# DanEngelbrecht/longtail

Hardware: AMD Instinct MI355X
Metric: ingest GB/s (chunk+hash+compress) (higher is better)
Workload: dtype u8/u32

## Files before the change

longtail_amd/csrc/ablations/k_buzhash_prefix_regs.inc:

```

template <int MODE, int WAVES>
__global__ __launch_bounds__(64 * WAVES, 1) void k_buzhash_prefix(const uint8_t* __restrict__ data,
                                                                   const PartDev* __restrict__ parts,
                                                                   const uint32_t* __restrict__ tile_part,
                                                                   uint32_t ntiles, DivTest dv,
                                                                   uint64_t* __restrict__ bm0,
                                                                   uint64_t* __restrict__ bm1)
{
    extern __shared__ __attribute__((aligned(16))) uint32_t smem[];
    const int tid = threadIdx.x;
    const int lane = tid & 63;
    const int wave = __builtin_amdgcn_readfirstlane(tid >> 6);
    uint32_t* rows = smem + 256 * TAB_REP + wave * (WROWS * ROW_DW + HALO_DW);
    uint32_t* halo = rows + WROWS * ROW_DW;
    prefix_table_init(smem, tid, 64 * WAVES);

    const uint32_t rows_byte = (uint32_t)(uintptr_t)(const __attribute__((address_space(3))) uint32_t*)rows;
    PrefixConsts pc;
    pc.lane4 = (uint32_t)lane * 4u;
    pc.hj = 63u - (uint32_t)lane;
    pc.halo_byte = rows_byte + WROWS * ROW_DW * 4u;
    pc.thr = MODE == 1 ? 0u : 0xFFFFFFFFu / (dv.d >> dv.k2);
    pc.exact_add = dv.addc - dv.inv;

    const uint64_t nwt = (uint64_t)ntiles * 4u;
    const uint64_t wstride = (uint64_t)gridDim.x * (uint64_t)WAVES;
    uint64_t wt = (uint64_t)blockIdx.x * (uint64_t)WAVES + (uint64_t)wave;
    if (wt >= nwt)
        return;
    PartDev pd = parts[tile_part[wt >> 2]];
    uint64_t span = ((wt >> 2) - pd.tile_base) * (uint64_t)TILE + (wt & 3u) * (uint64_t)WTILE;
    TileRegs regs;
    tile_load(regs, data, pd, span, lane);

    for (;;)
    {
        __builtin_amdgcn_wave_barrier();
        tile_store(regs, rows, lane);
        __builtin_amdgcn_wave_barrier();

        const uint64_t next = wt + wstride;
        PartDev npd = pd;
        uint64_t next_span = 0;
        if (next < nwt)
        {
            npd = parts[tile_part[next >> 2]];
            next_span = ((next >> 2) - npd.tile_base) * (uint64_t)TILE + (next & 3u) * (uint64_t)WTILE;
            tile_load(regs, data, npd, next_span, lane);
        }

        uint32_t win[16];
        const uint32_t* own = rows + (lane + 1) * ROW_DW;
#pragma unroll
        for (int i = 0; i < 16; ++i)
            win[i] = own[i];
        const uint32_t hb = lds_load_u8(rows_byte + pc.hj);
        const uint64_t m = prefix_legal(prefix_tile<MODE>(win, hb, pc, dv, lane, halo), span + (uint64_t)lane * RUN, pd.size);

        const uint64_t summary = __builtin_amdgcn_ballot_w64(m != 0ull);
        if (m != 0ull)
            bm0[pd.bm0_base + (span >> 6) + (uint64_t)lane] = m;
        if (lane == 0)
            bm1[pd.bm1_base + (span >> 12)] = summary;

        if (next >= nwt)
            break;
        wt = next;
        pd = npd;
        span = next_span;
    }
}
```

longtail_amd/csrc/ablations/k_buzhash_roll.inc:

```

constexpr int K1_WAVES = 12;
constexpr int K1_THREADS = 64 * K1_WAVES;
constexpr int WVECS = WROWS * 4;

struct TileRegs
{
    uint4 q[5];
};

__device__ __forceinline__ void tile_load(TileRegs& r, const uint8_t* __restrict__ data, const PartDev& pd,
                                          uint64_t span_start, int lane)
{
    const uint8_t* src = data + pd.off;
#pragma unroll
    for (int u = 0; u < 5; ++u)
    {
        const int v = lane + u * 64;
        uint4 q = make_uint4(0, 0, 0, 0);
        if (v < WVECS)
        {
            const int64_t g = (int64_t)span_start - 64 + 16 * (int64_t)v;
            if (g >= 0)
            {
                if ((uint64_t)g + 16 <= pd.size)
                    q = *reinterpret_cast<const uint4*>(src + g);
                else if ((uint64_t)g < pd.size)
                {
                    uint32_t w[4] = {0, 0, 0, 0};
                    const uint32_t n = (uint32_t)(pd.size - (uint64_t)g);
                    for (uint32_t b = 0; b < n; ++b)
                        w[b >> 2] |= (uint32_t)src[g + b] << (8 * (b & 3));
                    q = make_uint4(w[0], w[1], w[2], w[3]);
                }
            }
        }
        r.q[u] = q;
    }
}

__device__ __forceinline__ void tile_store(const TileRegs& r, uint32_t* __restrict__ rows, int lane)
{
#pragma unroll
    for (int u = 0; u < 5; ++u)
    {
        const int v = lane + u * 64;
        if (v < WVECS)
        {
            uint32_t* d = rows + (v >> 2) * ROW_DW + (v & 3) * 4;
            d[0] = r.q[u].x;
            d[1] = r.q[u].y;
            d[2] = r.q[u].z;
            d[3] = r.q[u].w;
        }
    }
}

template <int MODE>
__global__ __launch_bounds__(K1_THREADS, 1) void k_buzhash_candidates(const uint8_t* __restrict__ data,
                                                                       const PartDev* __restrict__ parts,
                                                                       const uint32_t* __restrict__ tile_part,
                                                                       uint32_t ntiles, DivTest dv,
                                                                       uint64_t* __restrict__ bm0,
                                                                       uint64_t* __restrict__ bm1)
{
    extern __shared__ __attribute__((aligned(16))) uint32_t smem[];
    uint32_t* tab = smem;

    const int tid = threadIdx.x;
    const int lane = tid & 63;
    const int wave = __builtin_amdgcn_readfirstlane(tid >> 6);
    uint32_t* rows = smem + 256 * TAB_REP + wave * (WROWS * ROW_DW);

    if (tid < 256)
    {
        const uint32_t tv = c_buztab[tid];
        uint4 q = make_uint4(tv, tv, tv, tv);
        uint4* dst = reinterpret_cast<uint4*>(tab + tid * TAB_REP);
#pragma unroll
        for (int j = 0; j < TAB_REP / 4; ++j)
            dst[j] = q;
    }
    __syncthreads();
    if ((uint32_t)(uintptr_t)(const __attribute__((address_space(3))) uint32_t*)smem != 0u)
        __builtin_trap();
    const uint32_t lane4 = (uint32_t)lane * 4u;
    const uint32_t qodd = MODE == 1 ? 0u : 0xFFFFFFFFu / (dv.d >> dv.k2);

    const uint64_t nwt = (uint64_t)ntiles * 4u;
    const uint64_t wstride = (uint64_t)gridDim.x * (uint64_t)K1_WAVES;
    uint64_t wt = (uint64_t)blockIdx.x * (uint64_t)K1_WAVES + (uint64_t)wave;
    if (wt >= nwt)
        return;
    PartDev pd = parts[tile_part[wt >> 2]];
    uint64_t span = ((wt >> 2) - pd.tile_base) * (uint64_t)TILE + (wt & 3u) * (uint64_t)WTILE;
    TileRegs regs;
    tile_load(regs, data, pd, span, lane);

    for (;;)
    {
        __builtin_amdgcn_wave_barrier();
        tile_store(regs, rows, lane);
        __builtin_amdgcn_wave_barrier();

        const uint64_t next = wt + wstride;
        PartDev npd = pd;
        uint64_t next_span = 0;
        if (next < nwt)
        {
            npd = parts[tile_part[next >> 2]];
            next_span = ((next >> 2) - npd.tile_base) * (uint64_t)TILE + (next & 3u) * (uint64_t)WTILE;
            tile_load(regs, data, npd, next_span, lane);
        }

        const uint64_t q0 = span + (uint64_t)lane * RUN;
        uint32_t mlo = 0, mhi = 0;
        if (q0 < pd.size)
        {
            uint32_t win[28];
            const uint32_t* prev = rows + lane * ROW_DW;
#pragma unroll
            for (int i = 0; i < 12; ++i)
                win[i] = prev[4 + i];
#pragma unroll
            for (int i = 0; i < 16; ++i)
                win[12 + i] = prev[ROW_DW + i];

            uint32_t tv[48 + RUN];
            uint32_t h = 0;
#define LT_LOOKUP(j)                                                                                                 \
    tv[j] = lds_load_u32(__builtin_amdgcn_perm(win[(j) >> 2], lane4, 0x0c0c0400u | ((uint32_t)((j) & 3) << 8)))
#define LT_STEP(k)                                                                                                   \
    {                                                                                                                \
        h = rotl32(h, 1) ^ rotl32(tv[k], 16) ^ tv[48 + (k)];                                                         \
        bool pre;                                                                                                    \
        if (MODE == 1)                                                                                               \
            pre = (h & (dv.d - 1u)) == dv.d - 1u;                                                                    \
        else         \
            pre = h * dv.inv + dv.inv <= qodd;                                                                       \
        if (__builtin_amdgcn_ballot_w64(pre) != 0ull)        \
        {                                                                                                            \
            asm volatile("");                  \
            const bool hit = MODE == 1 ? pre : rotr32(h * dv.inv + dv.addc, dv.k2) <= dv.qlim;    \
             \
            uint32_t hb;                                                                                             \
            asm volatile("v_cndmask_b32_e64 %0, 0, 1, %1" : "=v"(hb) : "s"(__builtin_amdgcn_ballot_w64(hit)));       \
            if ((k) < 32)                                                                                            \
                mlo |= hb << (k);                                                                                    \
            else                                                                                                     \
                mhi |= hb << ((k)-32);                                                                               \
        }                                                                                                            \
    }
#pragma unroll
            for (int j = 0; j < 80; ++j)
                LT_LOOKUP(j);
            __builtin_amdgcn_sched_barrier(0);
#pragma unroll
            for (int j = 0; j < 48; ++j)
                h = rotl32(h, 1) ^ tv[j];
#pragma unroll
            for (int k = 0; k < 32; ++k)
                LT_STEP(k)
            __builtin_amdgcn_sched_barrier(0);
#pragma unroll
            for (int j = 80; j < 48 + RUN; ++j)
                LT_LOOKUP(j);
            __builtin_amdgcn_sched_barrier(0);
#pragma unroll
            for (int k = 32; k < RUN; ++k)
                LT_STEP(k)
#undef LT_LOOKUP
#undef LT_STEP
            uint64_t m = ((uint64_t)mhi << 32) | mlo;
            if (q0 < 47)
                m &= ~0ull << (47 - q0);
            const uint64_t remain = pd.size - q0;
            if (remain < 64)
                m &= (1ull << remain) - 1ull;
            mlo = (uint32_t)m;
            mhi = (uint32_t)(m >> 32);
        }
        const uint64_t m = ((uint64_t)mhi << 32) | mlo;
        const uint64_t summary = __builtin_amdgcn_ballot_w64(m != 0ull);
        if (m != 0ull)
            bm0[pd.bm0_base + (span >> 6) + (uint64_t)lane] = m;
        if (lane == 0)
            bm1[pd.bm1_base + (span >> 12)] = summary;

        if (next >= nwt)
            break;
        wt = next;
        pd = npd;
        span = next_span;
    }
}
```

longtail_amd/csrc/k_buzhash.hip:

```cpp
#include "lthip_internal.h"

#include <stdlib.h>
#include <type_traits>

namespace
{

__constant__ uint32_t c_buztab[256] = {
#include "buzhash_table.inc"
};

#include "k_blake3_leaf.h"

constexpr int RUN = 64;
constexpr int TILE = 256 * RUN;
constexpr int ROW_DW = 17;
constexpr int TAB_REP = 64;

__device__ __forceinline__ uint32_t lds_load_u32(uint32_t byte_addr)
{
#if defined(__HIP_DEVICE_COMPILE__)
    return *(const __attribute__((address_space(3))) uint32_t*)byte_addr;
#else
    (void)byte_addr;
    return 0u;
#endif
}

__device__ __forceinline__ uint32_t lds_load_u8(uint32_t byte_addr)
{
#if defined(__HIP_DEVICE_COMPILE__)
    return *(const __attribute__((address_space(3))) uint8_t*)byte_addr;
#else
    (void)byte_addr;
    return 0u;
#endif
}

__device__ __forceinline__ uint4 lds_load_u128(uint32_t byte_addr)
{
#if defined(__HIP_DEVICE_COMPILE__)
    typedef uint32_t v4 __attribute__((ext_vector_type(4)));
    const v4 q = *(const __attribute__((address_space(3))) v4*)byte_addr;
    return make_uint4(q.x, q.y, q.z, q.w);
#else
    (void)byte_addr;
    return make_uint4(0, 0, 0, 0);
#endif
}

__device__ __forceinline__ uint32_t rotl32(uint32_t x, uint32_t r) { return __builtin_amdgcn_alignbit(x, x, (32u - r) & 31u); }
__device__ __forceinline__ uint32_t rotr32(uint32_t x, uint32_t r) { return __builtin_amdgcn_alignbit(x, x, r & 31u); }

__global__ void k_tile_table(const PartDev* __restrict__ parts, uint32_t nparts, uint32_t* __restrict__ tile_part,
                             uint64_t ntiles)
{
    uint64_t t = (uint64_t)blockIdx.x * blockDim.x + threadIdx.x;
    if (t >= ntiles)
        return;
    uint32_t lo = 0, hi = nparts;
    while (hi - lo > 1)
    {
        uint32_t mid = lo + (hi - lo) / 2;
        if ((uint64_t)parts[mid].tile_base <= t)
            lo = mid;
        else
            hi = mid;
    }
    tile_part[t] = lo;
}

constexpr int WROWS = 64 + 1;
constexpr int WTILE = 64 * RUN;

#ifdef LTHIP_ABLATIONS
#include "ablations/k_buzhash_roll.inc"
#endif

#ifndef K1_MAD64
#define K1_MAD64 0
#endif
constexpr int HALO_DW = 64;

struct PrefixConsts
{
    uint32_t lane4;
    uint32_t hj;
    uint32_t halo_byte;
    uint32_t thr;
    uint32_t exact_add;
};

template <int MODE>
__device__ __forceinline__ uint64_t prefix_tile(const uint32_t (&win)[16], uint32_t hb, const PrefixConsts& pc, const DivTest& dv,
                                                int lane, uint32_t* __restrict__ halo)
{
    {
        uint32_t x = lds_load_u32((hb << 8) | pc.lane4);
        x = rotr32(x, pc.hj);
        if (lane >= 47)
            x = 0u;
        x ^= (uint32_t)__builtin_amdgcn_update_dpp(0, (int)x, 0x111, 0xf, 0xf, false);
        x ^= (uint32_t)__builtin_amdgcn_update_dpp(0, (int)x, 0x112, 0xf, 0xf, false);
        x ^= (uint32_t)__builtin_amdgcn_update_dpp(0, (int)x, 0x114, 0xf, 0xf, false);
        x ^= (uint32_t)__builtin_amdgcn_update_dpp(0, (int)x, 0x118, 0xf, 0xf, false);
        x ^= (uint32_t)__builtin_amdgcn_update_dpp(0, (int)x, 0x142, 0xa, 0xf, false);
        x ^= (uint32_t)__builtin_amdgcn_update_dpp(0, (int)x, 0x143, 0xc, 0xf, false);
        halo[pc.hj] = x;
    }

    uint32_t S[65];
#define LT_LOOKUP(j) S[j] = lds_load_u32(__builtin_amdgcn_perm(win[(j) >> 2], pc.lane4, 0x0c0c0400u | ((uint32_t)((j) & 3) << 8)))
#pragma unroll
    for (int j = 63; j >= 0; --j)
        LT_LOOKUP(j);
#undef LT_LOOKUP
    __builtin_amdgcn_sched_barrier(0);
    S[64] = 0u;
#pragma unroll
    for (int j = 63; j >= 0; --j)
        S[j] = S[j + 1] ^ ((j & 31) ? rotr32(S[j], (uint32_t)(j & 31)) : S[j]);
    __builtin_amdgcn_wave_barrier();

    uint32_t mlo = 0, mhi = 0;
    uint32_t inv_v;
    asm volatile("v_mov_b32 %0, %1" : "=v"(inv_v) : "s"(dv.inv));
#if K1_MAD64
    const uint64_t inv64 = (uint64_t)inv_v;
#endif
    typedef uint32_t u32x4 __attribute__((ext_vector_type(4)));
    u32x4 Q[16];
    auto halo_quad = [&](auto QI) __attribute__((always_inline))
    {
        constexpr int q = decltype(QI)::value;
        if constexpr (q >= 4 && q <= 15)
        {
            u32x4 v = {S[4 * q], S[4 * q + 1], S[4 * q + 2], S[4 * q + 3]};
            uint64_t save;
            asm volatile("s_mov_b64 %[sv], exec\n\ts_mov_b64 exec, %[msk]\n\t"
                         "ds_read_b128 %[r], %[ad] offset:%[o]\n\t"
                         "s_mov_b64 exec, %[sv]"
                         : [sv] "=&s"(save), [r] "+v"(v)
                         : [ad] "v"(pc.halo_byte), [msk] "s"(0x8000000000000000ull), [o] "i"(16 * q)
                         : "memory");
            Q[q] = v;
        }
    };
    auto halo_wait = [&](auto QI) __attribute__((always_inline))
    {
        constexpr int q = decltype(QI)::value;
        if constexpr (q >= 4 && q <= 15)
        {
            u32x4 v = Q[q];
            if constexpr (q >= 6)
                asm volatile("s_waitcnt lgkmcnt(2)" : "+v"(v));
            else if constexpr (q == 5)
                asm volatile("s_waitcnt lgkmcnt(1)" : "+v"(v));
            else
                asm volatile("s_waitcnt lgkmcnt(0)" : "+v"(v));
            S[4 * q] = v.x;
            S[4 * q + 1] = v.y;
            S[4 * q + 2] = v.z;
            S[4 * q + 3] = v.w;
        }
    };
    auto group = [&](auto G) __attribute__((always_inline))
    {
        constexpr int g = decltype(G)::value;
        uint32_t y[8];
#pragma unroll
        for (int half = 1; half >= 0; --half)
        {
            if (half == 1)
                halo_wait(std::integral_constant<int, 2 * g + 1 + 4>{});
            else
                halo_wait(std::integral_constant<int, 2 * g + 4>{});
#pragma unroll
            for (int ii = 3; ii >= 0; --ii)
            {
                const int i = 4 * half + ii;
                const int k = 8 * g + i;
                uint32_t w;
                if (k >= 47)
                    w = S[k - 47] ^ S[k + 1];
                else
                    w = (S[0] ^ S[k + 1]) ^ (uint32_t)__builtin_amdgcn_update_dpp(0, (int)S[(k + 17) & 63], 0x13C, 0xf, 0xf, false);
                const uint32_t h = (k & 31) ? rotl32(w, (uint32_t)(k & 31)) : w;
                if (MODE == 1)
                    y[i] = ~h & (dv.d - 1u);
                else
                {
#if K1_MAD64
                    uint64_t t, carry;
                    asm("v_mad_u64_u32 %0, %1, %2, %3, %4" : "=v"(t), "=s"(carry) : "v"(h), "s"(dv.inv), "v"(inv64));
                    y[i] = (uint32_t)t;
#else
                    y[i] = h * dv.inv + inv_v;
#endif
                }
            }
            if (half == 1)
                halo_quad(std::integral_constant<int, 2 * g + 2>{});
            else
                halo_quad(std::integral_constant<int, 2 * g + 1>{});
        }
        const uint32_t m = min(min(min(y[0], y[1]), y[2]), min(min(min(y[3], y[4]), y[5]), min(y[6], y[7])));
        if (__builtin_amdgcn_ballot_w64(m <= pc.thr) != 0ull)
        {
            asm volatile("");
#pragma unroll
            for (int i = 0; i < 8; ++i)
            {
                const int k = 8 * g + i;
                if (__builtin_amdgcn_ballot_w64(y[i] <= pc.thr) != 0ull)
                {
                    asm volatile("");
                    const bool hit = MODE == 1 ? y[i] == 0u : rotr32(y[i] + pc.exact_add, dv.k2) <= dv.qlim;
                    uint32_t hbit;
                    asm volatile("v_cndmask_b32_e64 %0, 0, 1, %1" : "=v"(hbit) : "s"(__builtin_amdgcn_ballot_w64(hit)));
                    if (k < 32)
                        mlo |= hbit << k;
                    else
                        mhi |= hbit << (k - 32);
                }
            }
        }
    };
    group(std::integral_constant<int, 7>{});
    group(std::integral_constant<int, 6>{});
    group(std::integral_constant<int, 5>{});
    group(std::integral_constant<int, 4>{});
    group(std::integral_constant<int, 3>{});
    group(std::integral_constant<int, 2>{});
    group(std::integral_constant<int, 1>{});
    group(std::integral_constant<int, 0>{});
    return ((uint64_t)mhi << 32) | mlo;
}

__device__ __forceinline__ uint64_t prefix_legal(uint64_t m, uint64_t q0, uint64_t size)
{
    if (q0 >= size)
        return 0ull;
    if (q0 < 47)
        m &= ~0ull << (47 - q0);
    const uint64_t remain = size - q0;
    if (remain < 64)
        m &= (1ull << remain) - 1ull;
    return m;
}

__device__ __forceinline__ void prefix_table_init(uint32_t* tab, int tid, int nthreads)
{
    for (int v = tid; v < 256; v += nthreads)
    {
        const uint32_t tv = c_buztab[v];
        uint4 q = make_uint4(tv, tv, tv, tv);
        uint4* dst = reinterpret_cast<uint4*>(tab + v * TAB_REP);
#pragma unroll
        for (int j = 0; j < TAB_REP / 4; ++j)
            dst[j] = q;
    }
    __syncthreads();
    if ((uint32_t)(uintptr_t)(const __attribute__((address_space(3))) uint32_t*)tab != 0u)
        __builtin_trap();
}

#ifdef LTHIP_ABLATIONS
#include "ablations/k_buzhash_prefix_regs.inc"
#endif

constexpr int DMA_BUF_B = WROWS * 64;

constexpr int TAB_DW = 256 * TAB_REP;
constexpr int DMA_WAVE_DW = (DMA_BUF_B >> 2) + HALO_DW;
constexpr int PEND_CAP = 64;
constexpr size_t lds_tiles_dw(int waves) { return TAB_DW + (size_t)waves * DMA_WAVE_DW; }
constexpr size_t lds_pend_dw(int waves) { return lds_tiles_dw(waves); }
constexpr size_t lds_bytes(int waves, bool lists) { return sizeof(uint32_t) * lds_pend_dw(waves) + (lists ? sizeof(uint4) * waves * PEND_CAP : 0); }

struct WaveLds
{
    uint32_t* buf;
    uint32_t* halo;
    uint4* pend;
};
template <int WAVES>
__device__ __forceinline__ WaveLds wave_lds(uint32_t* smem, int wave)
{
    uint32_t* buf = smem + TAB_DW + wave * DMA_WAVE_DW;
    return {buf, buf + (DMA_BUF_B >> 2), reinterpret_cast<uint4*>(smem + lds_pend_dw(WAVES)) + wave * PEND_CAP};
}

struct TileDma
{
    const uint8_t* data;
    uint32_t* buf;
    int lane;
    uint32_t buf_byte;
    uint32_t buf_mid;
    uint32_t src_off;
    uint32_t own_row;
    uint32_t own_f;

    __device__ __forceinline__ TileDma(const uint8_t* d, uint32_t* b, int ln) : data(d), buf(b), lane(ln)
    {
        buf_byte = __builtin_amdgcn_readfirstlane((uint32_t)(uintptr_t)(const __attribute__((address_space(3))) uint32_t*)buf);
        buf_mid = buf_byte + 2048u;
        const uint32_t src_vec = 4u * ((uint32_t)lane >> 2) + (((uint32_t)lane & 3u) ^ (((uint32_t)lane >> 4) & 3u));
        src_off = 16u * src_vec;
        own_f = (((uint32_t)lane + 1u) >> 2) & 3u;
        own_row = buf_byte + 64u * ((uint32_t)lane + 1u);
    }

    template <int MODE>
    __device__ __forceinline__ PrefixConsts consts(const DivTest& dv) const
    {
        PrefixConsts pc;
        pc.lane4 = (uint32_t)lane * 4u;
        pc.hj = 63u - (uint32_t)lane;
        pc.halo_byte = buf_byte + DMA_BUF_B;
        pc.thr = MODE == 1 ? 0u : 0xFFFFFFFFu / (dv.d >> dv.k2);
        pc.exact_add = dv.addc - dv.inv;
        return pc;
    }

    template <int u>
    __device__ __forceinline__ void piece(const uint8_t* mid_src) const
    {
        asm volatile("s_mov_b32 m0, %[l]\n\ts_nop 0\n\t"
                     "global_load_lds_dwordx4 %[v], %[b] offset:%[o]"
                     :
                     : [v] "v"(src_off), [l] "s"(buf_mid), [b] "s"(mid_src), [o] "i"(1024 * u - 2048)
                     : "memory");
    }

    template <int u>
    __device__ __forceinline__ void edge(const PartDev& p, uint64_t sp, const uint8_t* mid_src) const
    {
        const int64_t base = (int64_t)sp - 64 + 1024 * u;
        const int64_t left = (int64_t)p.size - base;
        const int32_t left_hi = (int32_t)(left >> 32);
        const uint32_t before = base < 0 ? (uint32_t)-base : 0u;
        const uint32_t room = left_hi < 0 ? 0u : left_hi > 0 || (uint32_t)left > 1024u ? 1024u : (uint32_t)left;
        const uint32_t room16 = room & ~15u;
        const bool lane_on = (u < 4 || lane < 4) && src_off >= before;
        const bool whole = lane_on && src_off < room16;
        const bool part = lane_on && src_off == room16 && room != room16;
        if (whole)
            piece<u>(mid_src);
        if (part)
        {
            const uint8_t* src = mid_src + (1024 * u - 2048);
            uint32_t w[4] = {0, 0, 0, 0};
            const uint32_t n = room - src_off;
            for (uint32_t bb = 0; bb < n; ++bb)
                w[bb >> 2] |= (uint32_t)src[src_off + bb] << (8 * (bb & 3));
            uint32_t* d = buf + 256 * u + 4 * lane;
            d[0] = w[0];
            d[1] = w[1];
            d[2] = w[2];
            d[3] = w[3];
        }
    }

    __device__ __forceinline__ void issue(const PartDev& p, uint64_t sp) const
    {
        const uint8_t* mid_src = data + p.off + sp - 64 + 2048;
        if (sp >= 64 && sp + (uint64_t)WTILE <= p.size)
        {
            asm volatile("s_mov_b32 m0, %[l]\n\ts_nop 0\n\t"
                         "global_load_lds_dwordx4 %[v], %[b] offset:-2048\n\t"
                         "global_load_lds_dwordx4 %[v], %[b] offset:-1024\n\t"
                         "global_load_lds_dwordx4 %[v], %[b] offset:0\n\t"
                         "global_load_lds_dwordx4 %[v], %[b] offset:1024"
                         :
                         : [v] "v"(src_off), [l] "s"(buf_mid), [b] "s"(mid_src)
                         : "memory");
            if (lane < 4)
                piece<4>(mid_src);
        }
        else
        {
            edge<0>(p, sp, mid_src);
            edge<1>(p, sp, mid_src);
            edge<2>(p, sp, mid_src);
            edge<3>(p, sp, mid_src);
            edge<4>(p, sp, mid_src);
        }
    }

    __device__ __forceinline__ void take(uint32_t (&win)[16], uint32_t& hb, const PrefixConsts& pc) const
    {
        asm volatile("s_waitcnt vmcnt(0)" ::: "memory");
#pragma unroll
        for (int c = 0; c < 4; ++c)
        {
            const uint4 q = lds_load_u128(own_row + 16u * ((uint32_t)c ^ own_f));
            win[4 * c + 0] = q.x;
            win[4 * c + 1] = q.y;
            win[4 * c + 2] = q.z;
            win[4 * c + 3] = q.w;
        }
        hb = lds_load_u8(buf_byte + pc.hj);
        asm volatile("s_waitcnt lgkmcnt(0)" ::: "memory");
    }
};

__device__ __forceinline__ uint64_t* run_words(uint64_t* __restrict__ bm0, uint64_t first)
{
    uint64_t* w = bm0 + first;
    asm("" : "+s"(w));
    return w;
}

template <int MODE, int WAVES>
__global__ __launch_bounds__(64 * WAVES, 1) void k_buzhash_prefix_dma(const uint8_t* __restrict__ data,
                                                                       const PartDev* __restrict__ parts,
                                                                       const uint32_t* __restrict__ tile_part,
                                                                       uint32_t ntiles, DivTest dv,
                                                                       uint64_t* __restrict__ bm0,
                                                                       uint64_t* __restrict__ bm1)
{
    extern __shared__ __attribute__((aligned(16))) uint32_t smem[];
    const int tid = threadIdx.x;
    const int lane = tid & 63;
    const int wave = __builtin_amdgcn_readfirstlane(tid >> 6);
    const WaveLds lds = wave_lds<WAVES>(smem, wave);
    uint32_t* const halo = lds.halo;
    prefix_table_init(smem, tid, 64 * WAVES);

    const TileDma dma(data, lds.buf, lane);
    const PrefixConsts pc = dma.consts<MODE>(dv);

    const uint64_t nwt = (uint64_t)ntiles * 4u;
    const uint64_t wstride = (uint64_t)gridDim.x * (uint64_t)WAVES;
    uint64_t wt = (uint64_t)blockIdx.x * (uint64_t)WAVES + (uint64_t)wave;
    if (wt >= nwt)
        return;

    PartDev pd = parts[tile_part[wt >> 2]];
    uint64_t span = ((wt >> 2) - pd.tile_base) * (uint64_t)TILE + (wt & 3u) * (uint64_t)WTILE;
    dma.issue(pd, span);

    uint64_t pend_m = 0, pend_summary = 0, pend_i0 = 0, pend_i1 = 0;
    bool pend = false;
    for (;;)
    {
        uint32_t win[16], hb;
        dma.take(win, hb, pc);

        if (pend)
        {
            if (pend_m != 0ull)
                run_words(bm0, pend_i0)[(uint32_t)lane] = pend_m;
            if (lane == 0)
                bm1[pend_i1] = pend_summary;
        }

        const uint64_t next = wt + wstride;
        PartDev npd = pd;
        uint64_t next_span = 0;
        const bool more = (int64_t)(next - nwt) < 0;
        if (more)
        {
            npd = parts[tile_part[next >> 2]];
            next_span = ((next >> 2) - npd.tile_base) * (uint64_t)TILE + (next & 3u) * (uint64_t)WTILE;
            dma.issue(npd, next_span);
        }

        pend_m = prefix_legal(prefix_tile<MODE>(win, hb, pc, dv, lane, halo), span + (uint64_t)lane * RUN, pd.size);
        pend_summary = __builtin_amdgcn_ballot_w64(pend_m != 0ull);
        pend_i0 = pd.bm0_base + (span >> 6);
        pend_i1 = pd.bm1_base + (span >> 12);
        pend = true;

        if (!more)
            break;
        wt = next;
        pd = npd;
        span = next_span;
    }
    if (pend_m != 0ull)
        run_words(bm0, pend_i0)[(uint32_t)lane] = pend_m;
    if (lane == 0)
        bm1[pend_i1] = pend_summary;
}

__device__ __forceinline__ uint64_t bcast64(uint64_t v, int src_lane)
{
    uint32_t lo = __builtin_amdgcn_readlane((uint32_t)v, src_lane);
    uint32_t hi = __builtin_amdgcn_readlane((uint32_t)(v >> 32), src_lane);
    return ((uint64_t)hi << 32) | lo;
}

__global__ __launch_bounds__(64) void k_select_cuts(const PartDev* __restrict__ parts, uint32_t nparts,
                                                    const uint64_t* __restrict__ bm0, const uint64_t* __restrict__ bm1,
                                                    uint32_t min_chunk, uint32_t max_chunk, uint2* __restrict__ region,
                                                    uint32_t* __restrict__ part_count)
{
    const uint32_t p = blockIdx.x;
    if (p >= nparts)
        return;
    const int lane = threadIdx.x;
    const PartDev pd = parts[p];
    const uint64_t size = pd.size;
    const uint64_t* b0 = bm0 + pd.bm0_base;
    const uint64_t* b1 = bm1 + pd.bm1_base;
    uint2* out = region + pd.region_base;

    uint64_t s = 0;
    uint32_t n = 0;
    while (s < size)
    {
        const uint64_t left = size - s;
        uint64_t len;
        if (left <= min_chunk)
            len = left;
        else
        {
            const uint64_t end = left > max_chunk ? max_chunk : left;
            len = end;
            const uint64_t qlo = s + min_chunk;
            const uint64_t qhi = s + end - 1;
            if (qlo <= qhi)
            {
                const uint64_t rlo = qlo >> 6, rhi = qhi >> 6;
                const uint64_t wlo = rlo >> 6, whi = rhi >> 6;
                bool found = false;
                for (uint64_t w0 = wlo; w0 <= whi && !found; w0 += 64)
                {
                    const uint64_t w = w0 + (uint64_t)lane;
                    uint64_t word = 0;
                    if (w <= whi)
                    {
                        word = b1[w];
                        if (w == wlo)
                            word &= ~0ull << (rlo & 63);
                        if (w == whi && (rhi & 63) != 63)
                            word &= (1ull << ((rhi & 63) + 1)) - 1ull;
                    }
                    for (;;)
                    {
                        const uint64_t any = __builtin_amdgcn_ballot_w64(word != 0ull);
                        if (any == 0ull)
                            break;
                        const int f = __builtin_ctzll(any);
                        const uint64_t fw = bcast64(word, f);
                        const int bit = __builtin_ctzll(fw);
                        const uint64_t r = ((w0 + (uint64_t)f) << 6) + (uint64_t)bit;
                        uint64_t m = b0[r];
                        if (r == rlo)
                            m &= ~0ull << (qlo & 63);
                        if (r == rhi && (qhi & 63) != 63)
                            m &= (1ull << ((qhi & 63) + 1)) - 1ull;
                        if (m != 0ull)
                        {
                            const uint64_t q = (r << 6) + (uint64_t)__builtin_ctzll(m);
                            len = q - s + 1;
                            found = true;
                            break;
                        }
                        if (lane == f)
                            word &= word - 1ull;
                    }
                }
            }
        }
        if (lane == 0)
            out[n] = make_uint2((uint32_t)s, (uint32_t)len);
        ++n;
        s += len;
    }
    if (lane == 0)
        part_count[p] = n;
}

#ifdef LTHIP_ABLATIONS
__device__ unsigned long long g_walk_tiles;
#endif

template <int MODE, int WAVES, bool GUESS, bool HASH>
__device__ __forceinline__ void walk_body(const uint8_t* __restrict__ data, const PartDev* __restrict__ parts, uint32_t nparts, DivTest dv,
                                          uint32_t min_chunk, uint32_t max_chunk, uint2* __restrict__ region,
                                          uint32_t* __restrict__ part_count, uint32_t* __restrict__ ticket, uint32_t* __restrict__ cv_runs)
{
    extern __shared__ __attribute__((aligned(16))) uint32_t smem[];
    const int tid = threadIdx.x;
    const int lane = tid & 63;
    const WaveLds lds = wave_lds<WAVES>(smem, __builtin_amdgcn_readfirstlane(tid >> 6));
    uint32_t* const halo = lds.halo;
    [[maybe_unused]] uint4* const pend = lds.pend;
    prefix_table_init(smem, tid, 64 * WAVES);

    const TileDma dma(data, lds.buf, lane);
    const PrefixConsts pc = dma.consts<MODE>(dv);
    const int lane_base = lane * RUN;

    auto jump = [](uint64_t q) __attribute__((always_inline)) { return q >= 64 ? ((q - 64) & ~(uint64_t)15) + 64 : (uint64_t)0; };

    bool inflight = false;
    uint64_t inflight_tb = 0;
#ifdef LTHIP_ABLATIONS
    uint32_t tiles = 0;
#endif
    [[maybe_unused]] uint32_t pn = 0, pl = 0, phead = 0, last_nl = 0, slot = 0;
    bool have = false, scanning = false, drained = false;
    PartDev pd = {};
    uint32_t t = 0, n = 0, end = 0;
    uint64_t size = 0, s = 0, qlo = 0, qhi = 0, tb = 0;
    uint2* out = region;

    auto emit = [&](uint32_t len) __attribute__((always_inline))
    {
        if (lane == 0)
        {
            [[maybe_unused]] const uint64_t at = pd.off + s;
            out[n] = make_uint2((uint32_t)s, len);
            if constexpr (HASH)
                pend[pn] = make_uint4((uint32_t)at, (uint32_t)(at >> 32), len, slot);
        }
        if constexpr (HASH)
            last_nl = leaves_of(len);
        ++n;
        if constexpr (HASH)
        {
            ++pn;
            pl += last_nl;
            slot += last_nl;
        }
        s += len;
    };
    auto classify = [&](uint32_t& len) __attribute__((always_inline)) -> bool
    {
        const uint64_t left = size - s;
        len = left <= min_chunk ? (uint32_t)left : left > max_chunk ? max_chunk : (uint32_t)left;
        if (!(left > min_chunk && len > min_chunk))
            return false;
        end = len;
        qlo = s + min_chunk;
        qhi = s + end - 1;
        return true;
    };

    for (;;)
    {
        if constexpr (HASH)
            if (pl >= 64u || (drained && pl != 0u))
            {
                asm volatile("" ::: "memory");
                __builtin_amdgcn_wave_barrier();
                const bool has = (uint32_t)lane < pn;
                const uint4 e = pend[has ? lane : 0];
                const uint32_t cnt = has ? leaves_of(e.z) - (lane == 0 ? phead : 0u) : 0u;
                uint32_t incl = cnt;
                incl += (uint32_t)__builtin_amdgcn_update_dpp(0, (int)incl, 0x111, 0xf, 0xf, false);
                incl += (uint32_t)__builtin_amdgcn_update_dpp(0, (int)incl, 0x112, 0xf, 0xf, false);
                incl += (uint32_t)__builtin_amdgcn_update_dpp(0, (int)incl, 0x114, 0xf, 0xf, false);
                incl += (uint32_t)__builtin_amdgcn_update_dpp(0, (int)incl, 0x118, 0xf, 0xf, false);
                incl += (uint32_t)__builtin_amdgcn_update_dpp(0, (int)incl, 0x142, 0xa, 0xf, false);
                incl += (uint32_t)__builtin_amdgcn_update_dpp(0, (int)incl, 0x143, 0xc, 0xf, false);
                const uint32_t excl = incl - cnt;
                if (!has)
                    incl = 0xFFFFFFFFu;
                const uint32_t take = pl < 64u ? pl : 64u;
                uint32_t j = 0;
#pragma unroll
                for (uint32_t step = 32u; step; step >>= 1)
                    if ((uint32_t)__builtin_amdgcn_ds_bpermute((int)((j + step - 1u) * 4u), (int)incl) <= (uint32_t)lane)
                        j += step;
                const bool on = (uint32_t)lane < take;
                if (!on)
                    j = 0;
                const uint32_t k = (uint32_t)lane - (uint32_t)__builtin_amdgcn_ds_bpermute((int)(j * 4u), (int)excl) + (j == 0u ? phead : 0u);
                const uint4 c = pend[j];
                if (on)
                {
                    uint32_t cv[8];
                    b3_leaf(cv, data + (((uint64_t)c.y << 32) | c.x) + ((uint64_t)k << 10), c.z, k);
                    uint4* o = reinterpret_cast<uint4*>(cv_runs + (uint64_t)(c.w + k) * 8u);
                    o[0] = make_uint4(cv[0], cv[1], cv[2], cv[3]);
                    o[1] = make_uint4(cv[4], cv[5], cv[6], cv[7]);
                }
                pl -= take;
                if (pl != 0u)
                {
                    const uint32_t li = pn - 1u;
                    const uint4 l = make_uint4(__builtin_amdgcn_readlane(e.x, li), __builtin_amdgcn_readlane(e.y, li),
                                               __builtin_amdgcn_readlane(e.z, li), __builtin_amdgcn_readlane(e.w, li));
                    if (lane == 0)
                        pend[0] = l;
                    phead = last_nl - pl;
                    pn = 1;
                }
                else
                    pn = 0, phead = 0;
                asm volatile("" ::: "memory");
                __builtin_amdgcn_wave_barrier();
                continue;
            }
        if (drained)
            break;
        if (!have)
        {
            __builtin_amdgcn_wave_barrier();
            t = atomicAdd(ticket, lane == 0 ? 1u : 0u);
            t = __builtin_amdgcn_readfirstlane(t);
            if (t >= nparts)
            {
                drained = true;
                continue;
            }
            pd = parts[t];
            size = pd.size;
            out = region + pd.region_base;
            if constexpr (HASH)
                slot = (uint32_t)lthip_part_run_base(pd);
            s = 0;
            n = 0;
            have = true;
            scanning = false;
        }
        if (!scanning)
        {
            if (s >= size)
            {
                if (inflight)
                {
                    asm volatile("s_waitcnt vmcnt(0)" ::: "memory");
                    inflight = false;
                }
                if (lane == 0)
                    part_count[t] = n;
                have = false;
                continue;
            }
            uint32_t len;
            if (!classify(len))
            {
                emit(len);
                continue;
            }
            tb = jump(qlo);
            scanning = true;
        }

        auto ends_here = [&]() __attribute__((always_inline)) { return (uint32_t)(qhi - tb) < (uint32_t)WTILE; };
        if (!(inflight && inflight_tb == tb))
        {
            if (inflight)
                asm volatile("s_waitcnt vmcnt(0)" ::: "memory");
            dma.issue(pd, tb);
        }
        inflight = false;
        uint32_t win[16], hb;
        dma.take(win, hb, pc);
        if (GUESS)
        {
            uint64_t g = tb + (uint64_t)WTILE;
            bool aim = true;
            if (ends_here())
            {
                const uint64_t s2 = s + end;
                aim = size - s2 > min_chunk && max_chunk > min_chunk;
                g = jump(s2 + min_chunk);
            }
            if (aim)
            {
                dma.issue(pd, g);
                inflight = true;
                inflight_tb = g;
            }
        }
        const uint64_t raw = prefix_tile<MODE>(win, hb, pc, dv, lane, halo);
#ifdef LTHIP_ABLATIONS
        ++tiles;
#endif
        for (;;)
        {
            const int lo = (int)(qlo > tb ? qlo - tb : 0) - lane_base;
            const int hi = (int)(ends_here() ? (uint32_t)(qhi - tb) : (uint32_t)WTILE - 1u) - lane_base;
            uint64_t m = raw;
            if (lo > 0)
                m = lo > 63 ? 0ull : m & (~0ull << lo);
            if (hi < 63)
                m = hi < 0 ? 0ull : m & ((2ull << hi) - 1ull);
            const uint64_t any = __builtin_amdgcn_ballot_w64(m != 0ull);
            uint32_t len;
            if (any != 0ull)
            {
                const int f = __builtin_ctzll(any);
                const uint64_t q = tb + (uint64_t)(f * RUN + __builtin_ctzll(bcast64(m, f)));
                len = (uint32_t)(q - s) + 1u;
            }
            else if (ends_here())
                len = end;
            else
            {
                tb += (uint64_t)WTILE;
                break;
            }
            emit(len);
            uint32_t plain;
            if (s >= size || !classify(plain))
            {
                scanning = false;
                break;
            }
            if ((uint32_t)(qlo - tb) < (uint32_t)WTILE && (!HASH || pl < 64u))
                continue;
            tb = jump(qlo);
            break;
        }
    }
#ifdef LTHIP_ABLATIONS
    if (lane == 0 && tiles)
        atomicAdd(&g_walk_tiles, (unsigned long long)tiles);
#endif
}

template <int MODE, int WAVES, bool GUESS>
__global__ __launch_bounds__(64 * WAVES, 1) void k_buzhash_walk(const uint8_t* __restrict__ data, const PartDev* __restrict__ parts,
                                                                 uint32_t nparts, DivTest dv, uint32_t min_chunk, uint32_t max_chunk,
                                                                 uint2* __restrict__ region, uint32_t* __restrict__ part_count,
                                                                 uint32_t* __restrict__ ticket)
{
    walk_body<MODE, WAVES, GUESS, false>(data, parts, nparts, dv, min_chunk, max_chunk, region, part_count, ticket, nullptr);
}

template <int MODE, int WAVES, bool GUESS>
__global__ __launch_bounds__(64 * WAVES, 1) void k_buzhash_hash_walk(const uint8_t* __restrict__ data, const PartDev* __restrict__ parts,
                                                                      uint32_t nparts, DivTest dv, uint32_t min_chunk, uint32_t max_chunk,
                                                                      uint2* __restrict__ region, uint32_t* __restrict__ part_count,
                                                                      uint32_t* __restrict__ ticket, uint32_t* __restrict__ cv_runs)
{
    walk_body<MODE, WAVES, GUESS, true>(data, parts, nparts, dv, min_chunk, max_chunk, region, part_count, ticket, cv_runs);
}

constexpr int SCAN_THREADS = 256;
constexpr int SCAN_ITEMS = 8;
constexpr int SCAN_BLOCK = SCAN_THREADS * SCAN_ITEMS;

__device__ __forceinline__ uint32_t block_exclusive_scan(uint32_t v, uint32_t* total, uint32_t* sh )
{
    const int lane = threadIdx.x & 63, wave = threadIdx.x >> 6;
    uint32_t x = v;
#pragma unroll
    for (int o = 1; o < 64; o <<= 1)
    {
        uint32_t y = __shfl_up(x, o, 64);
        if (lane >= o)
            x += y;
    }
    if (lane == 63)
        sh[wave] = x;
    __syncthreads();
    uint32_t base = 0, tot = 0;
#pragma unroll
    for (int w = 0; w < SCAN_THREADS / 64; ++w)
    {
        uint32_t t = sh[w];
        if (w < wave)
            base += t;
        tot += t;
    }
    __syncthreads();
    *total = tot;
    return base + x - v;
}

__global__ __launch_bounds__(SCAN_THREADS) void k_scan_sums(const uint32_t* __restrict__ in, uint64_t n,
                                                            const uint32_t* __restrict__ n_dev,
                                                            uint32_t* __restrict__ sums)
{
    __shared__ uint32_t sh[8];
    if (n_dev)
        n = *n_dev < n ? *n_dev : n;
    const uint64_t base = (uint64_t)blockIdx.x * SCAN_BLOCK;
    uint32_t acc = 0;
#pragma unroll
    for (int i = 0; i < SCAN_ITEMS; ++i)
    {
        uint64_t idx = base + (uint64_t)i * SCAN_THREADS + threadIdx.x;
        if (idx < n)
            acc += in[idx];
    }
    uint32_t tot;
    block_exclusive_scan(acc, &tot, sh);
    if (threadIdx.x == 0)
        sums[blockIdx.x] = tot;
}

__global__ __launch_bounds__(SCAN_THREADS) void k_scan_spine(uint32_t* __restrict__ sums, uint32_t nblocks)
{
    __shared__ uint32_t sh[8];
    uint32_t carry = 0;
    for (uint32_t b0 = 0; b0 < nblocks; b0 += SCAN_THREADS)
    {
        uint32_t i = b0 + threadIdx.x;
        uint32_t v = i < nblocks ? sums[i] : 0;
        uint32_t tot;
        uint32_t ex = block_exclusive_scan(v, &tot, sh);
        if (i < nblocks)
            sums[i] = carry + ex;
        carry += tot;
    }
    if (threadIdx.x == 0)
        sums[nblocks] = carry;
}

__global__ __launch_bounds__(SCAN_THREADS) void k_scan_apply(const uint32_t* __restrict__ in, uint64_t n,
                                                             const uint32_t* __restrict__ n_dev,
                                                             const uint32_t* __restrict__ sums, uint32_t nblocks,
                                                             uint32_t* __restrict__ out)
{
    __shared__ uint32_t sh[8];
    if (n_dev)
        n = *n_dev < n ? *n_dev : n;
    const uint64_t base = (uint64_t)blockIdx.x * SCAN_BLOCK + (uint64_t)threadIdx.x * SCAN_ITEMS;
    uint32_t v[SCAN_ITEMS];
    uint32_t acc = 0;
#pragma unroll
    for (int i = 0; i < SCAN_ITEMS; ++i)
    {
        uint64_t idx = base + i;
        v[i] = idx < n ? in[idx] : 0;
        acc += v[i];
    }
    uint32_t tot;
    uint32_t ex = block_exclusive_scan(acc, &tot, sh) + sums[blockIdx.x];
#pragma unroll
    for (int i = 0; i < SCAN_ITEMS; ++i)
    {
        uint64_t idx = base + i;
        if (idx < n)
            out[idx] = ex;
        ex += v[i];
    }
    if (blockIdx.x == 0 && threadIdx.x == 0)
        out[n] = sums[nblocks];
}

__global__ __launch_bounds__(64) void k_compact_chunks(const PartDev* __restrict__ parts, uint32_t nparts,
                                                       const uint2* __restrict__ region,
                                                       const uint32_t* __restrict__ part_first,
                                                       uint64_t* __restrict__ chunk_offsets,
                                                       uint32_t* __restrict__ chunk_lens)
{
    const uint32_t p = blockIdx.x;
    if (p >= nparts)
        return;
    const PartDev pd = parts[p];
    const uint32_t first = part_first[p];
    const uint32_t n = part_first[p + 1] - first;
    const uint2* in = region + pd.region_base;
    for (uint32_t i = threadIdx.x; i < n; i += 64)
    {
        uint2 e = in[i];
        chunk_offsets[first + i] = pd.off + (uint64_t)e.x;
        chunk_lens[first + i] = e.y;
    }
}

__global__ __launch_bounds__(64) void k_chunk_from_buffer(const uint8_t* __restrict__ buf, uint32_t n, uint32_t min_chunk,
                                                          DivTest dv, uint64_t* __restrict__ out_len)
{
    const int lane = threadIdx.x;
    uint32_t h0 = 0;
    for (uint32_t i = 0; i < 48; ++i)
        h0 ^= rotl32(c_buztab[buf[i]], (47u - i) & 31u);
    uint32_t result = n;
    const uint32_t kmax = n - min_chunk;
    for (uint32_t k0 = 1; k0 <= kmax; k0 += 64)
    {
        const uint32_t k = k0 + (uint32_t)lane;
        bool hit = false;
        if (k <= kmax)
        {
            uint32_t h;
            if (k < 48)
            {
                h = rotl32(h0, k & 31u);
                for (uint32_t i = 1; i <= k; ++i)
                    h ^= rotl32(rotl32(c_buztab[buf[i - 1]], 16) ^ c_buztab[buf[min_chunk + i - 1]], (k - i) & 31u);
            }
            else
            {
                const uint32_t p = min_chunk + k;
                h = 0;
                for (uint32_t j = 0; j < 48; ++j)
                    h ^= rotl32(c_buztab[buf[p - 1 - j]], j & 31u);
            }
            hit = dv.pow2 ? (h & (dv.d - 1u)) == dv.d - 1u : rotr32(h * dv.inv + dv.addc, dv.k2) <= dv.qlim;
        }
        const uint64_t any = __builtin_amdgcn_ballot_w64(hit);
        if (any)
        {
            result = min_chunk + k0 + (uint32_t)__builtin_ctzll(any);
            break;
        }
    }
    if (lane == 0)
        *out_len = result;
}

}

int lthip_launch_from_buffer(lthip_ctx* ctx, const uint8_t* d_data, uint32_t n, uint32_t min_chunk, const DivTest& dv,
                             uint64_t* d_out)
{
    LaunchTimer t(ctx, LTHIP_K_OTHER);
    hipLaunchKernelGGL(k_chunk_from_buffer, dim3(1), dim3(64), 0, ctx->stream, d_data, n, min_chunk, dv, d_out);
    LTHIP_LAUNCH_CHECK(ctx);
    return 0;
}

int lthip_launch_tile_table(lthip_ctx* ctx, lthip_plan* plan)
{
    if (plan->ntiles == 0)
        return 0;
    LaunchTimer t(ctx, LTHIP_K_OTHER);
    const uint32_t blocks = (uint32_t)div_up_u64(plan->ntiles, 256);
    hipLaunchKernelGGL(k_tile_table, dim3(blocks), dim3(256), 0, ctx->stream, plan->d_parts, plan->nparts,
                       plan->d_tile_part, plan->ntiles);
    LTHIP_LAUNCH_CHECK(ctx);
    return 0;
}

#ifdef LTHIP_ABLATIONS
constexpr bool K1_HAS_REG_FLAVOUR = true;
#else
constexpr bool K1_HAS_REG_FLAVOUR = false;
#endif

template <int WAVES, bool DMA>
static int launch_buzhash_prefix(lthip_ctx* ctx, const lthip_plan* plan, const uint8_t* d_data, uint64_t* bm0, uint64_t* bm1)
{
    static_assert(DMA || K1_HAS_REG_FLAVOUR, "the register-staged flavour is compiled by the ablation build only");
    constexpr size_t lds = DMA ? lds_bytes(WAVES, false) : sizeof(uint32_t) * (256 * TAB_REP + WAVES * (WROWS * ROW_DW + HALO_DW));
    static_assert(lds <= 160 * 1024, "LDS budget: one workgroup per CU");
#ifdef LTHIP_ABLATIONS
    auto k0 = DMA ? &k_buzhash_prefix_dma<0, WAVES> : &k_buzhash_prefix<0, WAVES>;
    auto k1 = DMA ? &k_buzhash_prefix_dma<1, WAVES> : &k_buzhash_prefix<1, WAVES>;
#else
    auto k0 = &k_buzhash_prefix_dma<0, WAVES>;
    auto k1 = &k_buzhash_prefix_dma<1, WAVES>;
#endif
    static std::atomic<bool> granted[64] = {};
    if (int err = lthip_grant_lds(ctx, granted, {reinterpret_cast<const void*>(k0), reinterpret_cast<const void*>(k1)}, lds))
        return err;
    uint32_t grid = lthip_cu_count(ctx->device);
    if ((uint64_t)grid * WAVES > plan->ntiles * 4u)
        grid = (uint32_t)div_up_u64(plan->ntiles * 4u, WAVES);
    LaunchTimer t(ctx, LTHIP_K_BUZHASH);
    hipLaunchKernelGGL(plan->div.pow2 ? k1 : k0, dim3(grid), dim3(64 * WAVES), lds, ctx->stream, d_data, plan->d_parts,
                       plan->d_tile_part, (uint32_t)plan->ntiles, plan->div, bm0, bm1);
    LTHIP_LAUNCH_CHECK(ctx);
    return 0;
}

#ifdef LTHIP_ABLATIONS
static int k1_flavour()
{
    static std::atomic<int> f{-1};
    static std::atomic<uint32_t> seen{0};
    const uint32_t gen = g_lthip_env_gen;
    if (seen.load(std::memory_order_acquire) != gen)
    {
        const char* e = getenv("LTHIP_K1");
        f.store(!e ? 0 : !strcmp(e, "roll") ? 4 : !strcmp(e, "prefix12") ? 3 : !strcmp(e, "prefix16") ? 2 : !strcmp(e, "dma12") ? 1 : 0,
                std::memory_order_relaxed);
        seen.store(gen, std::memory_order_release);
    }
    return f.load(std::memory_order_relaxed);
}

static int launch_buzhash_roll(lthip_ctx* ctx, const lthip_plan* plan, const uint8_t* d_data, uint64_t* bm0, uint64_t* bm1)
{
    static_assert(sizeof(uint32_t) * (256 * TAB_REP + K1_WAVES * WROWS * ROW_DW) <= 160 * 1024, "LDS budget: one workgroup per CU");
    const size_t lds = sizeof(uint32_t) * (256 * TAB_REP + K1_WAVES * WROWS * ROW_DW);
    static std::atomic<bool> granted[64] = {};
    if (int err = lthip_grant_lds(ctx, granted, {reinterpret_cast<const void*>(&k_buzhash_candidates<0>), reinterpret_cast<const void*>(&k_buzhash_candidates<1>)}, lds))
        return err;
    uint32_t grid = lthip_cu_count(ctx->device);
    if ((uint64_t)grid * K1_WAVES > plan->ntiles * 4u)
        grid = (uint32_t)div_up_u64(plan->ntiles * 4u, K1_WAVES);
    LaunchTimer t(ctx, LTHIP_K_BUZHASH);
    if (plan->div.pow2)
        hipLaunchKernelGGL(k_buzhash_candidates<1>, dim3(grid), dim3(K1_THREADS), lds, ctx->stream, d_data, plan->d_parts,
                           plan->d_tile_part, (uint32_t)plan->ntiles, plan->div, bm0, bm1);
    else
        hipLaunchKernelGGL(k_buzhash_candidates<0>, dim3(grid), dim3(K1_THREADS), lds, ctx->stream, d_data, plan->d_parts,
                           plan->d_tile_part, (uint32_t)plan->ntiles, plan->div, bm0, bm1);
    LTHIP_LAUNCH_CHECK(ctx);
    return 0;
}
#endif

int lthip_launch_buzhash(lthip_ctx* ctx, const lthip_plan* plan, const uint8_t* d_data, uint64_t* bm0, uint64_t* bm1)
{
    if (plan->ntiles == 0)
        return 0;
#ifdef LTHIP_ABLATIONS
    const int flavour = k1_flavour();
    if (flavour == 1)
        return launch_buzhash_prefix<12, true>(ctx, plan, d_data, bm0, bm1);
    if (flavour == 2)
        return launch_buzhash_prefix<16, false>(ctx, plan, d_data, bm0, bm1);
    if (flavour == 3)
        return launch_buzhash_prefix<12, false>(ctx, plan, d_data, bm0, bm1);
    if (flavour == 4)
        return launch_buzhash_roll(ctx, plan, d_data, bm0, bm1);
#endif
    return launch_buzhash_prefix<16, true>(ctx, plan, d_data, bm0, bm1);
}

uint32_t lthip_cu_count(int device)
{
    static std::atomic<uint32_t> cached[64] = {};
    if (device >= 0 && device < 64 && cached[device].load(std::memory_order_relaxed))
        return cached[device].load(std::memory_order_relaxed);
    int ncu = 256;
    (void)hipDeviceGetAttribute(&ncu, hipDeviceAttributeMultiprocessorCount, device);
    const uint32_t n = (uint32_t)(ncu > 0 ? ncu : 256);
    if (device >= 0 && device < 64)
        cached[device].store(n, std::memory_order_relaxed);
    return n;
}

#ifndef K1_WALK_GUESS
#define K1_WALK_GUESS 1
#endif

template <int MODE, int WAVES, bool GUESS, bool HASH>
static constexpr auto walk_kernel()
{
    if constexpr (HASH)
        return &k_buzhash_hash_walk<MODE, WAVES, GUESS>;
    else
        return &k_buzhash_walk<MODE, WAVES, GUESS>;
}

template <bool GUESS, bool HASH>
static int launch_buzhash_walk(lthip_ctx* ctx, const lthip_plan* plan, const uint8_t* d_data, uint2* region, uint32_t* part_count,
                               uint32_t* cv_runs)
{
    constexpr int WAVES = 16;
    constexpr size_t lds = lds_bytes(WAVES, HASH);
    static_assert(lds <= 160 * 1024 && (sizeof(uint32_t) * lds_pend_dw(WAVES)) % 16 == 0,
                  "LDS budget: one workgroup per CU; the lists are 16-byte aligned");
    const auto k0 = walk_kernel<0, WAVES, GUESS, HASH>(), k1 = walk_kernel<1, WAVES, GUESS, HASH>();
    static std::atomic<bool> granted[64] = {};
    int err = lthip_grant_lds(ctx, granted, {reinterpret_cast<const void*>(k0), reinterpret_cast<const void*>(k1)}, lds);
    if (err)
        return err;
    void* ticket;
    if ((err = lthip_scratch(ctx, S_WALK_TICKET, 64, &ticket)))
        return err;
    uint32_t grid = lthip_cu_count(ctx->device);
    if ((uint64_t)grid * WAVES > plan->nparts)
        grid = (uint32_t)div_up_u64(plan->nparts, WAVES);
    LaunchTimer t(ctx, LTHIP_K_BUZHASH);
    LTHIP_CHECK(ctx, hipMemsetAsync(ticket, 0, 4, ctx->stream));
    const auto k = plan->div.pow2 ? k1 : k0;
    if constexpr (HASH)
        hipLaunchKernelGGL(k, dim3(grid), dim3(64 * WAVES), lds, ctx->stream, d_data, plan->d_parts, plan->nparts, plan->div,
                           plan->min_chunk, plan->max_chunk, region, part_count, (uint32_t*)ticket, cv_runs);
    else
        hipLaunchKernelGGL(k, dim3(grid), dim3(64 * WAVES), lds, ctx->stream, d_data, plan->d_parts, plan->nparts, plan->div,
                           plan->min_chunk, plan->max_chunk, region, part_count, (uint32_t*)ticket);
    LTHIP_LAUNCH_CHECK(ctx);
    return 0;
}

int lthip_launch_buzhash_walk(lthip_ctx* ctx, const lthip_plan* plan, const uint8_t* d_data, uint2* region, uint32_t* part_count,
                              uint32_t* cv_runs)
{
    if (plan->nparts == 0)
        return 0;
#ifdef LTHIP_ABLATIONS
    LTHIP_ABLATION_ENV(env_guess, "LTHIP_K1_WALK_GUESS");
    if (env_guess.get() >= 0 && (env_guess.get() != 0) != (K1_WALK_GUESS != 0))
        return cv_runs ? launch_buzhash_walk<!K1_WALK_GUESS, true>(ctx, plan, d_data, region, part_count, cv_runs)
                       : launch_buzhash_walk<!K1_WALK_GUESS, false>(ctx, plan, d_data, region, part_count, nullptr);
#endif
    return cv_runs ? launch_buzhash_walk<K1_WALK_GUESS != 0, true>(ctx, plan, d_data, region, part_count, cv_runs)
                   : launch_buzhash_walk<K1_WALK_GUESS != 0, false>(ctx, plan, d_data, region, part_count, nullptr);
}

extern "C" int lthip_debug_walk_tiles(uint64_t* out_tiles)
{
#ifdef LTHIP_ABLATIONS
    if (!out_tiles)
        return EINVAL;
    unsigned long long v = 0, zero = 0;
    if (hipDeviceSynchronize() != hipSuccess || hipMemcpyFromSymbol(&v, HIP_SYMBOL(g_walk_tiles), sizeof v) != hipSuccess ||
        hipMemcpyToSymbol(HIP_SYMBOL(g_walk_tiles), &zero, sizeof zero) != hipSuccess)
        return EIO;
    *out_tiles = v;
    return 0;
#else
    (void)out_tiles;
    return ENOTSUP;
#endif
}

int lthip_launch_select(lthip_ctx* ctx, const lthip_plan* plan, const uint64_t* bm0, const uint64_t* bm1, uint2* region,
                        uint32_t* part_count)
{
    LaunchTimer t(ctx, LTHIP_K_SELECT);
    hipLaunchKernelGGL(k_select_cuts, dim3(plan->nparts), dim3(64), 0, ctx->stream, plan->d_parts, plan->nparts, bm0, bm1,
                       plan->min_chunk, plan->max_chunk, region, part_count);
    LTHIP_LAUNCH_CHECK(ctx);
    return 0;
}

int lthip_exclusive_scan_u32(lthip_ctx* ctx, const uint32_t* d_in, uint32_t* d_out, uint64_t n_bound,
                             const uint32_t* d_n, int kid)
{
    const uint64_t nblocks64 = n_bound ? div_up_u64(n_bound, SCAN_BLOCK) : 1;
    if (nblocks64 > 0x7FFFFFFFull)
        return lthip_fail(ctx, EINVAL, "scan", "too many elements");
    const uint32_t nblocks = (uint32_t)nblocks64;
    void* tmp;
    int err = lthip_scratch(ctx, S_SCAN_TMP, ((size_t)nblocks + 1) * 4, &tmp);
    if (err)
        return err;
    uint32_t* sums = (uint32_t*)tmp;
    LaunchTimer t(ctx, kid);
    hipLaunchKernelGGL(k_scan_sums, dim3(nblocks), dim3(SCAN_THREADS), 0, ctx->stream, d_in, n_bound, d_n, sums);
    hipLaunchKernelGGL(k_scan_spine, dim3(1), dim3(SCAN_THREADS), 0, ctx->stream, sums, nblocks);
    hipLaunchKernelGGL(k_scan_apply, dim3(nblocks), dim3(SCAN_THREADS), 0, ctx->stream, d_in, n_bound, d_n, sums, nblocks,
                       d_out);
    LTHIP_LAUNCH_CHECK(ctx);
    return 0;
}

int lthip_launch_compact(lthip_ctx* ctx, const lthip_plan* plan, const uint2* region, const uint32_t* part_count,
                         uint32_t* d_part_first, uint64_t* d_chunk_offsets, uint32_t* d_chunk_lens)
{
    int err = lthip_exclusive_scan_u32(ctx, part_count, d_part_first, plan->nparts, nullptr, LTHIP_K_COMPACT);
    if (err || plan->nparts == 0)
        return err;
    LaunchTimer t(ctx, LTHIP_K_COMPACT);
    hipLaunchKernelGGL(k_compact_chunks, dim3(plan->nparts), dim3(64), 0, ctx->stream, plan->d_parts, plan->nparts, region,
                       (const uint32_t*)d_part_first, d_chunk_offsets, d_chunk_lens);
    LTHIP_LAUNCH_CHECK(ctx);
    return 0;
}
```

Baseline: 988.8.

## Store pre-rotated buzhash tables in LDS to drop per-lookup rotates

Replaces the 64-way replicated buzhash table with 32 pre-rotated copies (one per rotation amount), so each lookup reads the rotated value directly. The per-element rotr in the prefix XOR scan and the halo rotate disappear, and the address is formed with a single SDWA shift-by-byte instruction instead of a perm with lane offset. The LDS table also shrinks from 64 KB to 32 KB. In exchange, lanes no longer get their own private table copy, so LDS bank conflicts on lookups may increase.

```diff
diff --git a/longtail_amd/csrc/ablations/k_buzhash_prefix_regs.inc b/longtail_amd/csrc/ablations/k_buzhash_prefix_regs.inc
--- a/longtail_amd/csrc/ablations/k_buzhash_prefix_regs.inc
+++ b/longtail_amd/csrc/ablations/k_buzhash_prefix_regs.inc
@@ -11,13 +11,12 @@
     const int tid = threadIdx.x;
     const int lane = tid & 63;
     const int wave = __builtin_amdgcn_readfirstlane(tid >> 6);
-    uint32_t* rows = smem + 256 * TAB_REP + wave * (WROWS * ROW_DW + HALO_DW);
+    uint32_t* rows = smem + TAB_DW + wave * (WROWS * ROW_DW + HALO_DW);
     uint32_t* halo = rows + WROWS * ROW_DW;
     prefix_table_init(smem, tid, 64 * WAVES);
 
     const uint32_t rows_byte = (uint32_t)(uintptr_t)(const __attribute__((address_space(3))) uint32_t*)rows;
     PrefixConsts pc;
-    pc.lane4 = (uint32_t)lane * 4u;
     pc.hj = 63u - (uint32_t)lane;
     pc.halo_byte = rows_byte + WROWS * ROW_DW * 4u;
     pc.thr = MODE == 1 ? 0u : 0xFFFFFFFFu / (dv.d >> dv.k2);
diff --git a/longtail_amd/csrc/ablations/k_buzhash_roll.inc b/longtail_amd/csrc/ablations/k_buzhash_roll.inc
--- a/longtail_amd/csrc/ablations/k_buzhash_roll.inc
+++ b/longtail_amd/csrc/ablations/k_buzhash_roll.inc
@@ -1,4 +1,5 @@
 
+constexpr int TAB_REP = 64;
 constexpr int K1_WAVES = 12;
 constexpr int K1_THREADS = 64 * K1_WAVES;
 constexpr int WVECS = WROWS * 4;
diff --git a/longtail_amd/csrc/k_buzhash.hip b/longtail_amd/csrc/k_buzhash.hip
--- a/longtail_amd/csrc/k_buzhash.hip
+++ b/longtail_amd/csrc/k_buzhash.hip
@@ -15,7 +15,8 @@
 constexpr int RUN = 64;
 constexpr int TILE = 256 * RUN;
 constexpr int ROW_DW = 17;
-constexpr int TAB_REP = 64;
+constexpr int TAB_ROT = 32;
+constexpr int TAB_DW = TAB_ROT * 256;
 
 __device__ __forceinline__ uint32_t lds_load_u32(uint32_t byte_addr)
 {
@@ -84,20 +85,38 @@
 
 struct PrefixConsts
 {
-    uint32_t lane4;
     uint32_t hj;
     uint32_t halo_byte;
     uint32_t thr;
     uint32_t exact_add;
 };
 
+__device__ __forceinline__ uint32_t prefix_lookup(uint32_t w, int j)
+{
+    uint32_t a = 0;
+#if defined(__HIP_DEVICE_COMPILE__)
+#define LT_BYTE4(n) asm("v_lshlrev_b32_sdwa %0, 2, %1 dst_sel:DWORD dst_unused:UNUSED_PAD src0_sel:DWORD src1_sel:BYTE_" #n : "=v"(a) : "v"(w))
+    if ((j & 3) == 0)
+        LT_BYTE4(0);
+    else if ((j & 3) == 1)
+        LT_BYTE4(1);
+    else if ((j & 3) == 2)
+        LT_BYTE4(2);
+    else
+        LT_BYTE4(3);
+#undef LT_BYTE4
+#else
+    (void)w;
+#endif
+    return lds_load_u32(a + (uint32_t)(j & 31) * 1024u);
+}
+
 template <int MODE>
 __device__ __forceinline__ uint64_t prefix_tile(const uint32_t (&win)[16], uint32_t hb, const PrefixConsts& pc, const DivTest& dv,
                                                 int lane, uint32_t* __restrict__ halo)
 {
     {
-        uint32_t x = lds_load_u32((hb << 8) | pc.lane4);
-        x = rotr32(x, pc.hj);
+        uint32_t x = lds_load_u32(((pc.hj & 31u) << 10) + (hb << 2));
         if (lane >= 47)
             x = 0u;
         x ^= (uint32_t)__builtin_amdgcn_update_dpp(0, (int)x, 0x111, 0xf, 0xf, false);
@@ -110,16 +129,14 @@
     }
 
     uint32_t S[65];
-#define LT_LOOKUP(j) S[j] = lds_load_u32(__builtin_amdgcn_perm(win[(j) >> 2], pc.lane4, 0x0c0c0400u | ((uint32_t)((j) & 3) << 8)))
 #pragma unroll
     for (int j = 63; j >= 0; --j)
-        LT_LOOKUP(j);
-#undef LT_LOOKUP
+        S[j] = prefix_lookup(win[j >> 2], j);
     __builtin_amdgcn_sched_barrier(0);
     S[64] = 0u;
 #pragma unroll
     for (int j = 63; j >= 0; --j)
-        S[j] = S[j + 1] ^ ((j & 31) ? rotr32(S[j], (uint32_t)(j & 31)) : S[j]);
+        S[j] ^= S[j + 1];
     __builtin_amdgcn_wave_barrier();
 
     uint32_t mlo = 0, mhi = 0;
@@ -251,15 +268,8 @@
 
 __device__ __forceinline__ void prefix_table_init(uint32_t* tab, int tid, int nthreads)
 {
-    for (int v = tid; v < 256; v += nthreads)
-    {
-        const uint32_t tv = c_buztab[v];
-        uint4 q = make_uint4(tv, tv, tv, tv);
-        uint4* dst = reinterpret_cast<uint4*>(tab + v * TAB_REP);
-#pragma unroll
-        for (int j = 0; j < TAB_REP / 4; ++j)
-            dst[j] = q;
-    }
+    for (int i = tid; i < TAB_DW; i += nthreads)
+        tab[i] = rotr32(c_buztab[i & 255], (uint32_t)i >> 8);
     __syncthreads();
     if ((uint32_t)(uintptr_t)(const __attribute__((address_space(3))) uint32_t*)tab != 0u)
         __builtin_trap();
@@ -271,7 +281,6 @@
 
 constexpr int DMA_BUF_B = WROWS * 64;
 
-constexpr int TAB_DW = 256 * TAB_REP;
 constexpr int DMA_WAVE_DW = (DMA_BUF_B >> 2) + HALO_DW;
 constexpr int PEND_CAP = 64;
 constexpr size_t lds_tiles_dw(int waves) { return TAB_DW + (size_t)waves * DMA_WAVE_DW; }
@@ -316,7 +325,6 @@
     __device__ __forceinline__ PrefixConsts consts(const DivTest& dv) const
     {
         PrefixConsts pc;
-        pc.lane4 = (uint32_t)lane * 4u;
         pc.hj = 63u - (uint32_t)lane;
         pc.halo_byte = buf_byte + DMA_BUF_B;
         pc.thr = MODE == 1 ? 0u : 0xFFFFFFFFu / (dv.d >> dv.k2);
@@ -1036,7 +1044,7 @@
 static int launch_buzhash_prefix(lthip_ctx* ctx, const lthip_plan* plan, const uint8_t* d_data, uint64_t* bm0, uint64_t* bm1)
 {
     static_assert(DMA || K1_HAS_REG_FLAVOUR, "the register-staged flavour is compiled by the ablation build only");
-    constexpr size_t lds = DMA ? lds_bytes(WAVES, false) : sizeof(uint32_t) * (256 * TAB_REP + WAVES * (WROWS * ROW_DW + HALO_DW));
+    constexpr size_t lds = DMA ? lds_bytes(WAVES, false) : sizeof(uint32_t) * (TAB_DW + WAVES * (WROWS * ROW_DW + HALO_DW));
     static_assert(lds <= 160 * 1024, "LDS budget: one workgroup per CU");
 #ifdef LTHIP_ABLATIONS
     auto k0 = DMA ? &k_buzhash_prefix_dma<0, WAVES> : &k_buzhash_prefix<0, WAVES>;
```

Result: faster. 1002, median of 6 (+1.4%).
